# JingyangXiang/LLM-QAT

Hardware: AMD Instinct MI355X
Metric: fake-quant fwd+bwd Gelem/s & achieved HBM GB/s, 4096×11008 bf16 W4A8 (higher is better)
Workload: dtype bf16; 1 GPU; SymQuantizer fwd + STE bwd, W4 on weight-style [4096,11008] + A8 on activation-style [4096,11008], bf16, clip [-2,2] (LLaMA-7B W4-A8 down_proj shapes, configs[1]); parallelism=1gpu

## Files before the change

llm-qat_amd/csrc/fq_dtype_impl.h:

```cpp
#pragma once
#include "../../include/llmqat_fakequant.h"
#include "fq_launch.h"


namespace fq {

#define FQ_LAUNCH(kern, grid, block, st, ...) FQ_LAUNCHK(kern, dim3((unsigned)(grid)), dim3(block), 0, st, __VA_ARGS__)

template <int DT, bool ASYM, bool FAST, bool NTL, int NTS, bool DBG, bool PITCH = false>
static void launch_reg(const RowArgs& a, int64_t nvec, hipStream_t st) {
#define R(TPR, V)                                                                                                   \
    case V:                                                                                                         \
        FQ_LAUNCH((row_reg_kernel<DT, TPR, V, ASYM, FAST, NTL, NTS, DBG, 0, PITCH>), (TPR == 64 ? (a.rows + 3) / 4 : a.rows), \
                  (TPR == 64 ? 256 : TPR), st, a);                                                                  \
        break;
    if (nvec <= 192) {
        switch ((int)((nvec + 63) / 64)) { R(64, 1) R(64, 2) R(64, 3) }
    } else if (nvec <= 384) {
        switch ((int)((nvec + 127) / 128)) { R(128, 2) R(128, 3) }
    } else if (nvec <= 768) {
        switch ((int)((nvec + 255) / 256)) { R(256, 2) R(256, 3) }
    } else if (nvec <= 4096) {
        switch ((int)((nvec + 511) / 512)) { R(512, 2) R(512, 3) R(512, 4) case 5: R(512, 6) case 7: R(512, 8) }
    } else {
        switch ((int)((nvec + 1023) / 1024)) { case 5: R(1024, 6) case 7: R(1024, 8) }
    }
#undef R
}

template <int DT, int AC, bool NTL, bool NTS, bool PITCH = false>
static void launch_reg_ac(const RowArgs& a, int64_t nvec, hipStream_t st) {
#define R(TPR, V)                                                                                                            \
    case V:                                                                                                                  \
        FQ_LAUNCH((row_reg_kernel<DT, TPR, V, false, false, NTL, NTS, false, AC, PITCH>), (TPR == 64 ? (a.rows + 3) / 4 : a.rows),  \
                  (TPR == 64 ? 256 : TPR), st, a);                                                                           \
        break;
    if (nvec <= 192) {
        switch ((int)((nvec + 63) / 64)) { R(64, 1) R(64, 2) R(64, 3) }
    } else if (nvec <= 384) {
        switch ((int)((nvec + 127) / 128)) { R(128, 2) R(128, 3) }
    } else if (nvec <= 768) {
        switch ((int)((nvec + 255) / 256)) { R(256, 2) R(256, 3) }
    } else if (nvec <= 4096) {
        switch ((int)((nvec + 511) / 512)) { R(512, 2) R(512, 3) R(512, 4) case 5: R(512, 6) case 7: R(512, 8) }
    } else {
        switch ((int)((nvec + 1023) / 1024)) { case 5: R(1024, 6) case 7: R(1024, 8) }
    }
#undef R
}

template <int DT, int TPR, bool NTL, bool NTS, bool PITCH = false>
static void launch_wide(const RowArgs& a, int hpt, hipStream_t st) {
    const int64_t grid = TPR == 64 ? (a.rows + 3) / 4 : a.rows;
    constexpr int BLOCK = TPR == 64 ? 256 : TPR;
    const bool mask = any_mask(a) || PITCH;
    switch (hpt) {
#define H(N)                                                                                            \
    case N:                                                                                             \
        if (mask) FQ_LAUNCH((row_reg_wide_kernel<DT, TPR, N, NTL, NTS, true, PITCH>), grid, BLOCK, st, a);     \
        else if constexpr (!PITCH) FQ_LAUNCH((row_reg_wide_kernel<DT, TPR, N, NTL, NTS, false>), grid, BLOCK, st, a);         \
        break;
        H(1) H(2) H(3) H(4) H(5) H(6) case 7: H(8)
#undef H
        default: break;
    }
}

template <int DT, int AC>
static int sym_autocast_t(RowArgs a, void* ws, size_t wsb, hipStream_t st) {
    using T = Ty<DT>;
    begin_launches();
    seal_slots(a);
    if constexpr (T::ESIZE != 2) {
        return fail(FQ_ERR_DTYPE, "autocast arithmetic applies to bf16 / fp16 tensors only");
    } else {
        constexpr int EPV = 8;
        const bool pair = a.n_more > 0;
        const bool vec_ok = aligned16(a.x) && aligned16(a.y) && (a.cols % EPV == 0) && more_aligned(a, 15u, 15u) && pitches_aligned(a, 15, 15);
        const int64_t nvec = a.cols / EPV;
        const int64_t big_rows = largest_rows(a);
        const int64_t bytes = big_rows * a.cols * T::ESIZE;
        if (a.rows > 0x7FFFFFFF) return fail(FQ_ERR_SHAPE, "rows=%lld exceeds the grid limit", (long long)a.rows);
        const bool pitched = any_pitch(a);
        if constexpr (AC == 2) {
            const int64_t nh = a.cols / 4;
            const bool wide_ok = aligned16(a.y) && (reinterpret_cast<uintptr_t>(a.x) & 7u) == 0 && a.cols % 4 == 0 && nh <= 1024 * 8 &&
                                 more_aligned(a, 7u, 15u) && pitches_aligned(a, 7, 15);
            if (wide_ok) {
                const bool ntl = bytes >= NT_LOAD_MIN_BYTES;
#define W(TPR)                                                                                          \
    {                                                                                                   \
        const int hpt = (int)((nh + TPR - 1) / TPR);                                                    \
        if (pitched) launch_wide<DT, TPR, false, true, true>(a, hpt, st);                               \
        else if (ntl) launch_wide<DT, TPR, true, true>(a, hpt, st);                                     \
        else launch_wide<DT, TPR, false, true>(a, hpt, st);                                             \
    }
                if (nh <= 512) W(64) else if (nh <= 2048) W(256) else W(1024)
#undef W
                return launch_result();
            }
            if (pair || a.mask)
                return fail(FQ_ERR_UNSUPPORTED, "fp32-result forward with STE mask / second tensor: rows must be 8-byte aligned, cols %% 4 == 0, cols <= 32768");
            if (a.cols <= GENERIC_MAX_COLS) {
                if (a.cols <= 1024) FQ_LAUNCH((row_generic_kernel<DT, 64, false, AC>), (a.rows + 3) / 4, 256, st, a);
                else FQ_LAUNCH((row_generic_kernel<DT, 256, false, AC>), a.rows, 256, st, a);
                return launch_result();
            }
        } else {
            if (pair && !(vec_ok && nvec <= REG_MAX_VEC))
                return fail(FQ_ERR_UNSUPPORTED, "pair launch: rows must be 16-byte aligned and fit the register kernels");
        }
        if (AC == 1 && vec_ok && nvec <= REG_MAX_VEC) {
            if constexpr (AC == 1) {
                if (pitched) launch_reg_ac<DT, AC, false, true, true>(a, nvec, st);
                else if (bytes >= NT_LOAD_MIN_BYTES) launch_reg_ac<DT, AC, true, true>(a, nvec, st);
                else launch_reg_ac<DT, AC, false, true>(a, nvec, st);
            }
        } else if (a.mask) {
            return fail(FQ_ERR_UNSUPPORTED, "STE-mask forward needs 16-byte aligned rows that fit the register kernels");
        } else if (a.cols <= GENERIC_MAX_COLS) {
            if (a.cols <= 1024) FQ_LAUNCH((row_generic_kernel<DT, 64, false, AC>), (a.rows + 3) / 4, 256, st, a);
            else FQ_LAUNCH((row_generic_kernel<DT, 256, false, AC>), a.rows, 256, st, a);
        } else {
            if (pitched) return fail(FQ_ERR_UNSUPPORTED, "rows that do not follow one another: not served by the two-pass path");
            if (!ws || wsb < (size_t)a.rows * 8)
                return fail(FQ_ERR_WORKSPACE, "two-pass path needs %zu workspace bytes, got %zu", (size_t)a.rows * 8, wsb);
            if (hipMemsetAsync(ws, 0, (size_t)a.rows * 8, st) != hipSuccess) return fail(FQ_ERR_LAUNCH, "hipMemsetAsync failed");
            uint32_t* w = (uint32_t*)ws;
            const bool svec = aligned16(a.x) && a.cols % EPV == 0;
            const int64_t sch = svec ? tp_chunk_elems<DT, true>() : tp_chunk_elems<DT, false>();
            const int64_t schunks = (a.cols + sch - 1) / sch, ach = (int64_t)TP_THREADS * TP_EPT, achunks = (a.cols + ach - 1) / ach;
            if (a.rows * schunks > 0x7FFFFFFF || a.rows * achunks > 0x7FFFFFFF) return fail(FQ_ERR_SHAPE, "rows*chunks exceeds the grid limit");
            if (svec) FQ_LAUNCH((stats_kernel<DT, false, true>), a.rows * schunks, TP_THREADS, st, a, w, schunks);
            else FQ_LAUNCH((stats_kernel<DT, false, false>), a.rows * schunks, TP_THREADS, st, a, w, schunks);
            FQ_LAUNCH((apply_autocast_kernel<DT, AC == 2>), a.rows * achunks, TP_THREADS, st, a, (const uint32_t*)w, achunks);
        }
        return launch_result();
    }
}

template <int DT> int launch_sym_autocast(bool wide, RowArgs a, void* ws, size_t wsb, hipStream_t st) {
    return wide ? sym_autocast_t<DT, 2>(a, ws, wsb, st) : sym_autocast_t<DT, 1>(a, ws, wsb, st);
}

template <int DT, bool ASYM, bool FAST>
static int rowwise_t(RowArgs a, void* ws, size_t wsb, hipStream_t st) {
    using T = Ty<DT>;
    begin_launches();
    seal_slots(a);
    constexpr int EPV = 16 / T::ESIZE;
    const bool pair = a.n_more > 0;
    const bool vec_ok = aligned16(a.x) && aligned16(a.y) && (a.cols % EPV == 0) && more_aligned(a, 15u, 15u) && pitches_aligned(a, 15, 15);
    const int64_t nvec = a.cols / EPV;
    const int64_t big_rows = largest_rows(a);
    const int64_t bytes = big_rows * a.cols * T::ESIZE;
    const bool pitched = any_pitch(a);
    const bool ntl = bytes >= NT_LOAD_MIN_BYTES;
    bool two_pass = false, two_pass_vec = false;
    if (pair && !(vec_ok && nvec <= REG_MAX_VEC)) return fail(FQ_ERR_UNSUPPORTED, "pair launch: rows must be 16-byte aligned and fit the register kernels");
    if (vec_ok && nvec <= REG_MAX_VEC) {
        if (a.rows > 0x7FFFFFFF) return fail(FQ_ERR_SHAPE, "rows=%lld exceeds the grid limit", (long long)a.rows);
        if (a.idx || a.scale) launch_reg<DT, ASYM, FAST, false, false, true>(a, nvec, st);
        else if (pitched) launch_reg<DT, ASYM, FAST, false, true, false, true>(a, nvec, st);
        else if (ntl) launch_reg<DT, ASYM, FAST, true, ASYM ? ST_NT : ST_NT_SC1, false>(a, nvec, st);
        else launch_reg<DT, ASYM, FAST, false, true, false>(a, nvec, st);
    } else if (a.mask) {
        return fail(FQ_ERR_UNSUPPORTED, "STE-mask forward needs 16-byte aligned rows that fit the register kernels");
    } else if (vec_ok && !pitched) {
        two_pass = two_pass_vec = true;
    } else if (a.cols <= GENERIC_MAX_COLS) {
        if (a.rows > 0x7FFFFFFF) return fail(FQ_ERR_SHAPE, "rows=%lld exceeds the grid limit", (long long)a.rows);
        if (a.cols <= 1024) FQ_LAUNCH((row_generic_kernel<DT, 64, ASYM>), (a.rows + 3) / 4, 256, st, a);
        else FQ_LAUNCH((row_generic_kernel<DT, 256, ASYM>), a.rows, 256, st, a);
    } else {
        two_pass = true;
    }
    if (two_pass) {
        if (pitched) return fail(FQ_ERR_UNSUPPORTED, "rows that do not follow one another: not served by the two-pass path");
        if (!ws || wsb < (size_t)a.rows * 8)
// ... 90 lines not shown
    return blk;
}
#define FQ_LAUNCH2(kern, gx_, gy_, block, st, ...) FQ_LAUNCHK(kern, dim3((unsigned)(gx_), (unsigned)(gy_)), dim3(block), 0, st, __VA_ARGS__)

template <int DT> int launch_ste_mask(SteLaunch L, int64_t cols, float lo, float hi, hipStream_t st) {
    using T = Ty<DT>;
    begin_launches();
    constexpr int EPV = 16 / T::ESIZE;
    const int64_t mrw = mask_row_words(cols, T::ESIZE);
    if (!mrw) return fail(FQ_ERR_UNSUPPORTED, "STE-mask backward: shape not served");
    for (int i = 0; i < L.n; ++i)
        if (!(aligned16(L.t[i].g) && aligned16(L.t[i].gx) && (reinterpret_cast<uintptr_t>(L.t[i].mask) & 7u) == 0 && pitch_aligned(L.t[i].gp, 15) &&
              pitch_aligned(L.t[i].op, 15)))
            return fail(FQ_ERR_UNSUPPORTED, "STE-mask backward: alignment not served (g / gx rows 16 bytes, mask 8 bytes)");
    const int64_t nvec_row = cols / EPV;
    const int64_t chunks = (nvec_row + STE_THREADS * 8 - 1) / (STE_THREADS * 8);
    int cv = (int)((nvec_row + chunks - 1) / chunks);
    cv = (cv + 63) / 64 * 64;
    const int vpt = (cv + STE_THREADS - 1) / STE_THREADS;
    const int64_t grid = ste_layout(L, true);
    if (grid > 0x7FFFFFFF) return fail(FQ_ERR_SHAPE, "rows exceed the grid limit");
    int64_t big_rows = 0;
    for (int i = 0; i < L.n; ++i)
        if (!L.t[i].inplace && L.t[i].rows > big_rows) big_rows = L.t[i].rows;
    const int64_t bytes = big_rows * cols * T::ESIZE;
    const bool ntl = bytes >= NT_LOAD_MIN_BYTES;
    bool pitched = false;
    for (int i = 0; i < L.n; ++i) pitched = pitched || L.t[i].gp.on || L.t[i].op.on;
    if (L.n == 1 && !L.t[0].inplace && !pitched) {
        const SteSlot& t0 = L.t[0];
#define S1(V)                                                                                                                                            \
    case V:                                                                                                                                              \
        if (ntl) FQ_LAUNCH2((ste_mask_one_kernel<DT, V, true, true>), grid, chunks, STE_THREADS, st, t0.g, t0.gx, t0.bounds, t0.mask, nvec_row, cv, mrw, lo, hi);   \
        else FQ_LAUNCH2((ste_mask_one_kernel<DT, V, false, true>), grid, chunks, STE_THREADS, st, t0.g, t0.gx, t0.bounds, t0.mask, nvec_row, cv, mrw, lo, hi);      \
        break;
        switch (vpt) { S1(1) S1(2) S1(3) S1(4) S1(5) S1(6) S1(7) S1(8) }
#undef S1
        return launch_result();
    }
    if (L.n <= 2 && !pitched) {
#define S2(V)                                                                                                                  \
    case V:                                                                                                                    \
        if (ntl) FQ_LAUNCH2((ste_mask_kernel<DT, V, true, ST_NT_SC1, false, 2>), grid, chunks, STE_THREADS, st, L, nvec_row, cv, mrw, lo, hi);   \
        else FQ_LAUNCH2((ste_mask_kernel<DT, V, false, true, false, 2>), grid, chunks, STE_THREADS, st, L, nvec_row, cv, mrw, lo, hi);      \
        break;
        switch (vpt) { S2(1) S2(2) S2(3) S2(4) S2(5) S2(6) S2(7) S2(8) }
#undef S2
        return launch_result();
    }
#define S(V)                                                                                                               \
    case V:                                                                                                                \
        if (pitched) FQ_LAUNCH2((ste_mask_kernel<DT, V, false, true, true>), grid, chunks, STE_THREADS, st, L, nvec_row, cv, mrw, lo, hi);   \
        else if (ntl) FQ_LAUNCH2((ste_mask_kernel<DT, V, true, true>), grid, chunks, STE_THREADS, st, L, nvec_row, cv, mrw, lo, hi);        \
        else FQ_LAUNCH2((ste_mask_kernel<DT, V, false, true>), grid, chunks, STE_THREADS, st, L, nvec_row, cv, mrw, lo, hi);           \
        break;
    switch (vpt) { S(1) S(2) S(3) S(4) S(5) S(6) S(7) S(8) }
#undef S
    return launch_result();
}

template <int DT> int launch_ste_mask_wide(SteLaunch L, int64_t cols, float lo, float hi, hipStream_t st) {
    using T = Ty<DT>;
    begin_launches();
    if constexpr (T::ESIZE != 2) {
        return fail(FQ_ERR_DTYPE, "fp32-gradient STE backward applies to bf16 / fp16 inputs only");
    } else {
        const int64_t mrw = mask_row_words(cols, T::ESIZE);
        auto al8 = [](const void* p) { return (reinterpret_cast<uintptr_t>(p) & 7u) == 0; };
        if (!mrw || cols > 32768) return fail(FQ_ERR_UNSUPPORTED, "fp32-gradient STE backward: shape not served");
        for (int i = 0; i < L.n; ++i)
            if (!(aligned16(L.t[i].g) && al8(L.t[i].gx) && al8(L.t[i].mask) && pitch_aligned(L.t[i].gp, 15) && pitch_aligned(L.t[i].op, 7)))
                return fail(FQ_ERR_UNSUPPORTED, "fp32-gradient STE backward: alignment not served");
        const int64_t nh_row = cols / 4;
        const int64_t chunks = (nh_row + STE_THREADS * 8 - 1) / (STE_THREADS * 8);
        int ch = (int)((nh_row + chunks - 1) / chunks);
        ch = (ch + 63) / 64 * 64;
        const int hpt = (ch + STE_THREADS - 1) / STE_THREADS;
        const int64_t grid = ste_layout(L, false);
        if (grid > 0x7FFFFFFF) return fail(FQ_ERR_SHAPE, "rows exceed the grid limit");
        const int64_t bytes = largest_rows(L) * cols * 4;
        const bool ntl = bytes >= NT_LOAD_MIN_BYTES;
        bool pitched = false;
        for (int i = 0; i < L.n; ++i) pitched = pitched || L.t[i].gp.on || L.t[i].op.on;
        if (!ntl && !pitched && L.n <= 2) {
#define SN(V)                                                                                                                                  \
    case V:                                                                                                                                    \
        if (L.n == 1) FQ_LAUNCH2((ste_mask_wide_kernel<DT, V, false, true, false, 1>), grid, chunks, STE_THREADS, st, L, nh_row, ch, mrw, lo, hi);        \
        else FQ_LAUNCH2((ste_mask_wide_kernel<DT, V, false, true, false, 2>), grid, chunks, STE_THREADS, st, L, nh_row, ch, mrw, lo, hi);                 \
        break;
            switch (hpt) { SN(1) SN(2) SN(3) SN(4) SN(5) SN(6) SN(7) SN(8) }
#undef SN
            return launch_result();
        }
#define S(V)                                                                                                                  \
    case V:                                                                                                                   \
        if (pitched) FQ_LAUNCH2((ste_mask_wide_kernel<DT, V, false, true, true>), grid, chunks, STE_THREADS, st, L, nh_row, ch, mrw, lo, hi);   \
        else if (ntl) FQ_LAUNCH2((ste_mask_wide_kernel<DT, V, true, true>), grid, chunks, STE_THREADS, st, L, nh_row, ch, mrw, lo, hi);        \
        else FQ_LAUNCH2((ste_mask_wide_kernel<DT, V, false, true>), grid, chunks, STE_THREADS, st, L, nh_row, ch, mrw, lo, hi);           \
        break;
        switch (hpt) { S(1) S(2) S(3) S(4) S(5) S(6) S(7) S(8) }
#undef S
        return launch_result();
    }
}

template <int DT>
int launch_w12(const void* w, const void* scale, void* out, int64_t rows, int64_t cols, int w_bits, int scale_per_row, float cv,
               hipStream_t st) {
    using T = Ty<DT>;
    begin_launches();
    constexpr int EPV = 16 / T::ESIZE;
    const bool vec = aligned16(w) && aligned16(out) && cols % EPV == 0;
    int64_t grid = vec ? (rows * (cols / EPV) + 255) / 256 : (rows * cols + 255) / 256;
    if (!vec && grid > 16384) grid = 16384;
    if (grid > 0x7FFFFFFF) return fail(FQ_ERR_SHAPE, "tensor too large");
    if (w_bits == 1) {
        if (vec) FQ_LAUNCH((w12_kernel<DT, 1, true>), grid, 256, st, w, scale, out, rows, cols, scale_per_row, cv);
        else FQ_LAUNCH((w12_kernel<DT, 1, false>), grid, 256, st, w, scale, out, rows, cols, scale_per_row, cv);
    } else {
        if (vec) FQ_LAUNCH((w12_kernel<DT, 2, true>), grid, 256, st, w, scale, out, rows, cols, scale_per_row, cv);
        else FQ_LAUNCH((w12_kernel<DT, 2, false>), grid, 256, st, w, scale, out, rows, cols, scale_per_row, cv);
    }
    return launch_result();
}

template <int DT>
int launch_w12_rows(const void* w, void* out, void* scale_out, int64_t rows, int64_t cols, int w_bits, float cv, hipStream_t st) {
    using T = Ty<DT>;
    if (!(aligned16(w) && aligned16(out) && cols % 4 == 0 && cols >= 256 && rows >= 8))
        return fail(FQ_ERR_UNSUPPORTED, "one-launch 1-/2-bit branch: needs rows >= 8, cols >= 256, cols %% 4 == 0 and 16-byte aligned tensors");
    if (rows > 0x7FFFFFFF) return fail(FQ_ERR_SHAPE, "rows=%lld exceeds the grid limit", (long long)rows);
    const int64_t ngroups = cols / 4;
    const bool shared_row = cols >= 8129;
    const int64_t gpt = shared_row ? (ngroups + 511) / 512 : (ngroups + 63) / 64;
    constexpr int MAXG_OWN = DT == F32 ? 16 : 32;
    if (gpt > (shared_row ? 16 : MAXG_OWN) || (shared_row && (cols + 511) / 512 >= 256))
        return fail(FQ_ERR_UNSUPPORTED, "one-launch 1-/2-bit branch: cols=%lld outside the row lengths this kernel holds in registers", (long long)cols);
    begin_launches();
    const float factor = (float)rows / (float)(rows * cols);
    const bool ntl = rows * cols * T::ESIZE >= NT_LOAD_MIN_BYTES;
    const int64_t grid = shared_row ? rows : (rows + 7) / 8;
#define K(SH, G, WB)                                                                                                              \
    {                                                                                                                             \
        if (ntl) FQ_LAUNCH((w12_row_aten_kernel<DT, WB, SH, G, true, true>), grid, 512, st, w, out, scale_out, rows, cols, cv, factor);   \
        else FQ_LAUNCH((w12_row_aten_kernel<DT, WB, SH, G, false, true>), grid, 512, st, w, out, scale_out, rows, cols, cv, factor);      \
    }
#define KW(SH, G)                    \
    {                                \
        if (w_bits == 1) K(SH, G, 1) \
        else K(SH, G, 2)             \
    }
    if (shared_row) {
        if (gpt <= 6) KW(true, 6) else if (gpt <= 8) KW(true, 8) else KW(true, 16)
    } else {
        if (gpt <= 16) KW(false, 16)
        else if constexpr (DT != F32) KW(false, 32)
    }
#undef KW
#undef K
    return launch_result();
}

#define FQ_INSTANTIATE(DT)                                                                                      \
    template int launch_rowwise<DT>(bool, bool, RowArgs, void*, size_t, hipStream_t);                           \
    template int launch_sym_autocast<DT>(bool, RowArgs, void*, size_t, hipStream_t);                                           \
    template int launch_ste<DT>(const void*, const void*, void*, int64_t, float, float, hipStream_t);           \
    template int launch_ste_rows<DT>(const void*, const void*, void*, int64_t, int64_t, float, float, const float*, hipStream_t, const StePitch3&); \
    template int launch_ste_mask<DT>(SteLaunch, int64_t, float, float, hipStream_t);                             \
    template int launch_ste_mask_wide<DT>(SteLaunch, int64_t, float, float, hipStream_t);                        \
    template int launch_w12<DT>(const void*, const void*, void*, int64_t, int64_t, int, int, float, hipStream_t);     \
    template int launch_w12_rows<DT>(const void*, void*, void*, int64_t, int64_t, int, float, hipStream_t);

}
```

llm-qat_amd/csrc/fq_kernels.h:

```cpp
#pragma once
#include "fq_device.h"



namespace fq {

constexpr int MAX_MORE = 3;

struct RowPitch {
    int64_t outer, inner;
    uint32_t n_inner;
    uint32_t on;
};
template <bool PITCH = true> __device__ __forceinline__ int64_t row_byte_off(int64_t row, int64_t row_bytes, const RowPitch& p) {
    if constexpr (!PITCH) {
        return row * row_bytes;
    } else {
        if (!p.on) return row * row_bytes;
        const uint32_t r = (uint32_t)row, q = r / p.n_inner;
        return (int64_t)q * p.outer + (int64_t)(r - q * p.n_inner) * p.inner;
    }
}

struct TensorSlot {
// ... 228 lines not shown
    }

    const bool want_mask = msk && !((ub < a.hi) && (lb > a.lo));
    const bool sym_clip = a.lo == -a.hi;
    const uint32_t clipk = (ub != ub) ? 0u : a.clipk;
    uint8_t* mrow = (uint8_t*)(msk + row * a.mask_row_words);
    int32_t* idxr = (DBG && a.idx) ? a.idx + row * a.cols : nullptr;
#pragma unroll
    for (int i = 0; i < VPT; ++i) {
        const int v = t + i * TPR;
        const uint32_t w[4] = {r[i].x, r[i].y, r[i].z, r[i].w};
        float f[EPV];
#pragma unroll
        for (int d = 0; d < 4; ++d) {
            float fd[T::EPD];
            T::unpack(w[d], fd);
#pragma unroll
            for (int k = 0; k < T::EPD; ++k) f[d * T::EPD + k] = fd[k];
        }
        if (want_mask) ste_mask_record<DT>(mrow, v, v < nvec, r[i], f, a.lo, a.hi, sym_clip, clipk);
        if constexpr (AC != 0) {
#pragma unroll
            for (int e = 0; e < EPV; ++e) f[e] = sym_elem_autocast(f[e], sr);
            uint32_t o[4];
#pragma unroll
            for (int d = 0; d < 4; ++d) {
                float fd[T::EPD];
#pragma unroll
                for (int k = 0; k < T::EPD; ++k) fd[k] = f[d * T::EPD + k];
                o[d] = T::pack(fd);
            }
            if (v < nvec) st16_at<NTS>(yr, v, make_uint4(o[0], o[1], o[2], o[3]));
            continue;
        }
        uint32_t o[4];
        int32_t ib[EPV];
#pragma unroll
        for (int d = 0; d < 4; ++d) {
            float fd[T::EPD];
#pragma unroll
            for (int k = 0; k < T::EPD; ++k) fd[k] = f[d * T::EPD + k];
            int32_t* ip = (DBG && idxr) ? ib + d * T::EPD : nullptr;
            if constexpr (!ASYM) o[d] = sym_chain<DT, FAST>(fd, sr, ip);
            else if constexpr (ALUT) {
                if (use_lut) {
                    const uint16_t* L = lut[TPR == 64 ? (threadIdx.x >> 6) : 0];
                    const uint32_t i0 = as_u(asym_first_half<DT, AFAST>(fd[0], ar, a.asym) + 12582912.0f) & 0xFFu;
                    const uint32_t i1 = as_u(asym_first_half<DT, AFAST>(fd[1], ar, a.asym) + 12582912.0f) & 0xFFu;
                    o[d] = (uint32_t)L[i0] | ((uint32_t)L[i1] << 16);
                } else {
                    o[d] = asym_chain<DT, AFAST>(fd, ar, a.asym, ip);
                }
            } else o[d] = asym_chain<DT, FAST && DT == BF16>(fd, ar, a.asym, ip);
        }
        if (v < nvec) {
            st16_at<NTS>(yr, v, make_uint4(o[0], o[1], o[2], o[3]));
            if constexpr (DBG) {
                if (idxr) {
#pragma unroll
                    for (int e = 0; e < EPV; ++e) idxr[(int64_t)v * EPV + e] = ib[e];
                }
            }
        }
    }
}

typedef uint32_t u32x2_t __attribute__((ext_vector_type(2)));
template <bool NT> __device__ __forceinline__ uint2 ld8(const uint2* p) {
    if constexpr (NT) {
        u32x2_t v = __builtin_nontemporal_load((const u32x2_t*)p);
        return make_uint2(v.x, v.y);
    } else {
        return *p;
    }
}
template <bool NT> __device__ __forceinline__ void st8(uint2* p, uint2 v) {
    if constexpr (NT) {
        u32x2_t w = {v.x, v.y};
        __builtin_nontemporal_store(w, (u32x2_t*)p);
    } else {
        *p = v;
    }
}

template <int DT, int TPR, int HPT, bool NTL, bool NTS, bool MASK, bool PITCH = false>
__global__ __launch_bounds__(TPR == 64 ? 256 : TPR) void row_reg_wide_kernel(RowArgs a) {
    using T = Ty<DT>;
    static_assert(T::ESIZE == 2, "16-bit input, fp32 output");
    constexpr int NW = TPR / 64;
    __shared__ uint32_t red[NW > 1 ? NW : 1];
    int64_t row;
    int t;
    if constexpr (TPR == 64) {
        row = (int64_t)blockIdx.x * 4 + (threadIdx.x >> 6);
        t = threadIdx.x & 63;
        if (row >= a.rows) return;
    } else {
        row = blockIdx.x;
        t = threadIdx.x;
    }
    const void* xb = a.x;
    void* yb = a.y;
    float* bnd = a.bounds;
    uint64_t* msk = a.mask;
    float qmax = a.sym.qmax;
    RowPitch xp = a.xp, yp = a.yp;
    if (row >= a.rows0) {
        int64_t rbase = 0;
#pragma unroll
        for (int i = 0; i < MAX_MORE; ++i) {
            if (i < a.n_more && row >= a.more[i].row_begin) {
                rbase = a.more[i].row_begin;
                xb = a.more[i].x;
                yb = a.more[i].y;
                bnd = a.more[i].bounds;
                msk = a.more[i].mask;
                qmax = a.more[i].qmax;
                if constexpr (PITCH) {
                    xp = a.more[i].xp;
                    yp = a.more[i].yp;
                }
            }
        }
        row -= rbase;
    }
    const int nh = (int)(a.cols / 4);
    const uint2* __restrict__ xr = (const uint2*)((const char*)xb + row_byte_off<PITCH>(row, a.cols * 2, xp));
    uint4* __restrict__ yr = (uint4*)((char*)yb + row_byte_off<PITCH>(row, a.cols * 4, yp));
    uint2 r[HPT];
#pragma unroll
    for (int i = 0; i < HPT; ++i) {
        int h = t + i * TPR;
        h = h < nh ? h : nh - 1;
        r[i] = ld8<NTL>(&xr[h]);
    }
    uint32_t acc = 0;
#pragma unroll
    for (int i = 0; i < HPT; ++i) acc = T::absmax_acc(T::absmax_acc(acc, r[i].x), r[i].y);
    const float m = as_f(block_reduce<OpMaxU, NW>(T::absmax_finish(acc), red));
    const SymRow sr = sym_row_autocast<DT>(m, SymConst{qmax, a.sym.c6});
    if (t == 0 && bnd) {
        bnd[2 * row] = m;
        bnd[2 * row + 1] = -m;
    }
    const bool want_mask = MASK && msk && !((m < a.hi) && (-m > a.lo));
    const bool sym_clip = a.lo == -a.hi;
    const uint32_t clipk = (m != m) ? 0u : a.clipk;
    uint8_t* mrow = (uint8_t*)(msk + row * a.mask_row_words);
#pragma unroll
    for (int i = 0; i < HPT; ++i) {
        const int h = t + i * TPR;
        float f[4];
        {
            float f0[2], f1[2];
            T::unpack(r[i].x, f0);
            T::unpack(r[i].y, f1);
            f[0] = f0[0], f[1] = f0[1], f[2] = f1[0], f[3] = f1[1];
        }
        if (MASK && want_mask) {
            uint32_t nib;
            if (clipk) nib = ste_flags16_pair(r[i].x, r[i].y, clipk);
            else nib = sym_clip ? ste_flags_f<4, true>(f, a.lo, a.hi) : ste_flags_f<4, false>(f, a.lo, a.hi);
            nib = h < nh ? nib : 0u;
            const uint32_t byte = ste_nibble_pair(nib);
            if (h < nh && !(h & 1)) mrow[h >> 1] = (uint8_t)byte;
        }
        const uint4 o = make_uint4(as_u(sym_elem_autocast(f[0], sr)), as_u(sym_elem_autocast(f[1], sr)),
                                   as_u(sym_elem_autocast(f[2], sr)), as_u(sym_elem_autocast(f[3], sr)));
        if (h < nh) st16<NTS>(&yr[h], o);
    }
}

template <int DT, bool FAST> __device__ __forceinline__ float sym_elem(float x, const SymRow& r, int32_t* idx) {
    using T = Ty<DT>;
    float q = __builtin_rintf(T::rb(x * r.s));
    if (idx) *idx = idx_i32(q);
    return FAST ? q * r.rinv : q / r.t2;
}
template <int DT> __device__ __forceinline__ float asym_elem(float x, const AsymRow& r, const AsymConst& k, int32_t* idx) {
    using T = Ty<DT>;
    float n = T::rb(T::rb(x - r.mn) / r.a);
    float q = __builtin_rintf(T::rb(n * k.S));
    if (idx) *idx = idx_i32(q);
    float w = T::rb(k.mul_inv ? q * k.invS : q / k.S);
    return T::rb(w * r.a) + r.mn;
}

template <int DT, int TPR, bool ASYM, int AC = 0>
__global__ __launch_bounds__(TPR == 64 ? 256 : TPR) void row_generic_kernel(RowArgs a) {
    using T = Ty<DT>;
    static_assert(AC == 0 || (!ASYM && T::ESIZE == 2), "autocast arithmetic: Sym on 16-bit tensors");
    constexpr int NW = TPR / 64;
    __shared__ uint32_t red[3][NW > 1 ? NW : 1];
    int64_t row;
    int t;
    if constexpr (TPR == 64) {
        row = (int64_t)blockIdx.x * 4 + (threadIdx.x >> 6);
        t = threadIdx.x & 63;
        if (row >= a.rows) return;
    } else {
        row = blockIdx.x;
        t = threadIdx.x;
    }
    const int64_t base = row * a.cols;
    const int64_t cols = a.cols;
    const int64_t xbase = row_byte_off(row, cols * T::ESIZE, a.xp) / T::ESIZE;
    const int64_t ybase = row_byte_off(row, cols * (AC == 2 ? 4 : T::ESIZE), a.yp) / (AC == 2 ? 4 : T::ESIZE);
    const float first = T::load1(a.x, xbase);
    SymRow sr;
    AsymRow ar;
    if constexpr (!ASYM) {
        uint32_t acc = 0;
        for (int64_t c = t; c < cols; c += TPR) {
            uint32_t b = as_u(T::load1(a.x, xbase + c)) & 0x7FFFFFFFu;
            acc = acc > b ? acc : b;
        }
        const float m = as_f(block_reduce<OpMaxU, NW>(acc, red[0]));
        if constexpr (AC == 0) sr = sym_row<DT>(m, a.sym);
        else sr = sym_row_autocast<DT>(m, a.sym);
        if (t == 0) {
            if (a.scale) a.scale[row] = sr.s;
            if (a.bounds) {
                a.bounds[2 * row] = m;
                a.bounds[2 * row + 1] = -m;
            }
        }
    } else {
        float mx = first, mn = first;
        uint32_t acc = 0;
        for (int64_t c = t; c < cols; c += TPR) {
            float v = T::load1(a.x, xbase + c);
            mx = __builtin_fmaxf(mx, v);
            mn = __builtin_fminf(mn, v);
            uint32_t b = as_u(v) & 0x7FFFFFFFu;
            acc = acc > b ? acc : b;
        }
        const uint32_t nb = block_reduce<OpMaxU, NW>(acc, red[0]);
        mx = as_f(block_reduce<OpMaxF, NW>(as_u(mx), red[1]));
        mn = as_f(block_reduce<OpMinF, NW>(as_u(mn), red[2]));
        if (absbits_is_nan(nb)) mx = mn = as_f(0x7FC00000u);
        ar = asym_row<DT>(mx, mn, a.asym);
        if (t == 0) {
            if (a.scale) {
                a.scale[2 * row] = ar.al;
                a.scale[2 * row + 1] = ar.mn;
            }
            if (a.bounds) {
                a.bounds[2 * row] = mx;
                a.bounds[2 * row + 1] = mn;
            }
        }
    }
// ... 520 lines not shown
                                               int64_t vs, int cv, const float* bounds, float lo, float hi, int t, const RowPitch& gp,
                                               const RowPitch& op) {
    using T = Ty<DT>;
    const uint4* gr = (const uint4*)((const char*)g + row_byte_off<PITCH>(row, nvec_row * 16, gp)) + vs;
    uint4* or_ = (uint4*)((char*)gx + row_byte_off<PITCH>(row, nvec_row * 16, op)) + vs;
    const int64_t rem = nvec_row - vs;
    const int nvec = (int)(rem < cv ? rem : cv);
    uint4 rg[VPT];
#pragma unroll
    for (int i = 0; i < VPT; ++i) {
        int v = t + i * STE_THREADS;
        v = v < nvec ? v : nvec - 1;
        rg[i] = ld16<NTL>(&gr[v]);
    }
    SteMaskHeld<16 / T::ESIZE, VPT> mh;
    mh.load(mrow, vs, mrow_dwords, t);
    bool safe = false;
    if (bounds) {
        const float ub = bounds[2 * row], lb = bounds[2 * row + 1];
        safe = (ub < hi) && (lb > lo);
    }
    if (safe) {
#pragma unroll
        for (int i = 0; i < VPT; ++i) {
            const int v = t + i * STE_THREADS;
            if (v < nvec) st16_at<NTS>(or_, v, rg[i]);
        }
    } else {
        uint32_t mb[VPT];
        mh.bits(t, mb);
#pragma unroll
        for (int i = 0; i < VPT; ++i) {
            const int v = t + i * STE_THREADS;
            const uint4 o = ste_mask_apply<DT>(rg[i], mb[i]);
            if (v < nvec) st16_at<NTS>(or_, v, o);
        }
    }
}

template <int DT, int VPT, bool NTL = true, bool NTS = true>
__global__ __launch_bounds__(STE_THREADS) void ste_mask_one_kernel(const void* g, void* gx, const float* bounds, const uint64_t* mask, int64_t nvec_row, int cv,
                                                                   int64_t mask_row_words, float lo, float hi) {
    const int64_t row = blockIdx.x;
    ste_mask_chunk<DT, VPT, NTL, NTS, false>(g, gx, (const uint8_t*)(mask + row * mask_row_words), (int)mask_row_words * 2, row, nvec_row, (int64_t)blockIdx.y * cv, cv,
                                             bounds, lo, hi, (int)threadIdx.x, RowPitch{}, RowPitch{});
}

template <int DT, int VPT, bool NTL = true, int NTS = ST_NT, bool PITCH = false, int NS = 4>
__global__ __launch_bounds__(STE_THREADS) void ste_mask_kernel(SteLaunch L, int64_t nvec_row, int cv, int64_t mask_row_words, float lo, float hi) {
    __shared__ uint64_t unsafe_rows[STE_THREADS / 64];
    const int t = threadIdx.x;
    const SteSlot sl = ste_pick_slot<PITCH, NS>(L, (int64_t)blockIdx.x);
    const int64_t local = (int64_t)blockIdx.x - sl.blk_begin;
    if (!sl.inplace) {
        ste_mask_chunk<DT, VPT, NTL, NTS, PITCH>(sl.g, sl.gx, (const uint8_t*)(sl.mask + local * mask_row_words), (int)mask_row_words * 2, local, nvec_row,
                                          (int64_t)blockIdx.y * cv, cv, sl.bounds, lo, hi, t, sl.gp, sl.op);
        return;
    }
    if (blockIdx.y) return;
    const int64_t r0 = local * STE_THREADS;
    bool unsafe = false;
    if (r0 + t < sl.rows) {
        const float ub = sl.bounds[2 * (r0 + t)], lb = sl.bounds[2 * (r0 + t) + 1];
        unsafe = !((ub < hi) && (lb > lo));
    }
    const uint64_t bal = __ballot(unsafe);
    if ((t & 63) == 0) unsafe_rows[t >> 6] = bal;
    __syncthreads();
#pragma unroll 1
    for (int w = 0; w < STE_THREADS / 64; ++w) {
        uint64_t bits = unsafe_rows[w];
        while (bits) {
            const int64_t row = r0 + w * 64 + __builtin_ctzll(bits);
            bits &= bits - 1;
            const uint8_t* mrow = (const uint8_t*)(sl.mask + row * mask_row_words);
#pragma unroll 1
            for (int c = 0; c < (int)gridDim.y; ++c)
                ste_mask_chunk<DT, VPT, false, false, PITCH>(sl.g, sl.gx, mrow, (int)mask_row_words * 2, row, nvec_row, (int64_t)c * cv, cv, nullptr, lo, hi, t,
                                                      sl.gp, sl.op);
        }
    }
}

template <int DT, int HPT, bool NTL = true, bool NTS = true, bool PITCH = false, int NS = 4>
__global__ __launch_bounds__(STE_THREADS) void ste_mask_wide_kernel(SteLaunch L, int64_t nh_row, int ch, int64_t mask_row_words, float lo, float hi) {
    using T = Ty<DT>;
    static_assert(T::ESIZE == 2, "fp32 gradient in, 16-bit gradient out");
    typedef short s16x2_t __attribute__((ext_vector_type(2)));
    SteSlot sl;
    if constexpr (NS == 1) sl = L.t[0];
    else sl = ste_pick_slot<PITCH, NS>(L, (int64_t)blockIdx.x);
    const int64_t row = (int64_t)blockIdx.x - sl.blk_begin;
    const int64_t hs = (int64_t)blockIdx.y * ch;
    const uint4* gr = (const uint4*)((const char*)sl.g + row_byte_off<PITCH>(row, nh_row * 16, sl.gp)) + hs;
    uint2* or_ = (uint2*)((char*)sl.gx + row_byte_off<PITCH>(row, nh_row * 8, sl.op)) + hs;
    const int64_t rem = nh_row - hs;
    const int nh = (int)(rem < ch ? rem : ch);
    const int t = threadIdx.x;
    uint4 rg[HPT];
#pragma unroll
    for (int i = 0; i < HPT; ++i) {
        int h = t + i * STE_THREADS;
        h = h < nh ? h : nh - 1;
        rg[i] = ld16<NTL>(&gr[h]);
    }
    SteMaskHeld<4, HPT> mh;
    mh.load((const uint8_t*)(sl.mask + row * mask_row_words), hs, (int)mask_row_words * 2, t);
    const float ub = sl.bounds[2 * row], lb = sl.bounds[2 * row + 1];
    const bool safe = (ub < hi) && (lb > lo);
    uint32_t mb[HPT];
    if (!safe) mh.bits(t, mb);
    else {
#pragma unroll
        for (int i = 0; i < HPT; ++i) mb[i] = 0u;
    }
#pragma unroll
    for (int i = 0; i < HPT; ++i) {
        const int h = t + i * STE_THREADS;
        const float f0[2] = {as_f(rg[i].x), as_f(rg[i].y)}, f1[2] = {as_f(rg[i].z), as_f(rg[i].w)};
        uint32_t w0 = T::pack(f0), w1 = T::pack(f1);
        const uint32_t m2 = mb[i] | (mb[i] << 15);
        w0 &= ~__builtin_bit_cast(uint32_t, __builtin_bit_cast(s16x2_t, m2 << 15) >> (short)15);
        w1 &= ~__builtin_bit_cast(uint32_t, __builtin_bit_cast(s16x2_t, m2 << 13) >> (short)15);
        if (h < nh) st8<NTS>(&or_[h], make_uint2(w0, w1));
    }
}

}
```

Measured before the change: 782.5 Gelem/s.

## Widen fake-quant forward loads and STE backward stores to 16 bytes via lane exchange

Result: no change. 783.5 Gelem/s, median of 6 (+0.1%).

```diff
diff --git a/llm-qat_amd/csrc/fq_dtype_impl.h b/llm-qat_amd/csrc/fq_dtype_impl.h
--- a/llm-qat_amd/csrc/fq_dtype_impl.h
+++ b/llm-qat_amd/csrc/fq_dtype_impl.h
@@ -49,16 +49,42 @@
 #undef R
 }
 
-template <int DT, int TPR, bool NTL, bool NTS, bool PITCH = false>
-static void launch_wide(const RowArgs& a, int hpt, hipStream_t st) {
+#ifndef FQ_WIDE_ST_BIG
+#define FQ_WIDE_ST_BIG ST_NT_SC1
+#endif
+#ifndef FQ_WIDE_ST_SMALL
+#define FQ_WIDE_ST_SMALL ST_NT
+#endif
+
+template <int DT, bool NTL, int NTS, bool PITCH = false>
+static void launch_wide(const RowArgs& a, int64_t nvec, hipStream_t st) {
+    const bool mask = any_mask(a) || PITCH;
+#define R(TPR, V)                                                                                                                          \
+    case V: {                                                                                                                              \
+        const int64_t grid = TPR == 64 ? (a.rows + 3) / 4 : a.rows;                                                                        \
+        if (mask) FQ_LAUNCH((row_reg_wide_kernel<DT, TPR, 2 * V, NTL, NTS, true, PITCH>), grid, (TPR == 64 ? 256 : TPR), st, a);           \
+        else if constexpr (!PITCH) FQ_LAUNCH((row_reg_wide_kernel<DT, TPR, 2 * V, NTL, NTS, false>), grid, (TPR == 64 ? 256 : TPR), st, a); \
+    } break;
+    if (nvec <= 192) {
+        switch ((int)((nvec + 63) / 64)) { R(64, 1) R(64, 2) R(64, 3) }
+    } else if (nvec <= 384) {
+        switch ((int)((nvec + 127) / 128)) { R(128, 2) R(128, 3) }
+    } else if (nvec <= 768) {
+        switch ((int)((nvec + 255) / 256)) { R(256, 2) R(256, 3) }
+    } else {
+        switch ((int)((nvec + 511) / 512)) { R(512, 2) R(512, 3) R(512, 4) case 5: R(512, 6) case 7: R(512, 8) }
+    }
+#undef R
+}
+
+template <int DT, int TPR>
+static void launch_wide_h8(const RowArgs& a, int hpt, hipStream_t st) {
     const int64_t grid = TPR == 64 ? (a.rows + 3) / 4 : a.rows;
     constexpr int BLOCK = TPR == 64 ? 256 : TPR;
-    const bool mask = any_mask(a) || PITCH;
     switch (hpt) {
-#define H(N)                                                                                            \
-    case N:                                                                                             \
-        if (mask) FQ_LAUNCH((row_reg_wide_kernel<DT, TPR, N, NTL, NTS, true, PITCH>), grid, BLOCK, st, a);     \
-        else if constexpr (!PITCH) FQ_LAUNCH((row_reg_wide_kernel<DT, TPR, N, NTL, NTS, false>), grid, BLOCK, st, a);         \
+#define H(N)                                                                                                   \
+    case N:                                                                                                    \
+        FQ_LAUNCH((row_reg_wide_kernel<DT, TPR, N, false, ST_NT, true, true, false>), grid, BLOCK, st, a);     \
         break;
         H(1) H(2) H(3) H(4) H(5) H(6) case 7: H(8)
 #undef H
@@ -88,13 +114,13 @@
                                  more_aligned(a, 7u, 15u) && pitches_aligned(a, 7, 15);
             if (wide_ok) {
                 const bool ntl = bytes >= NT_LOAD_MIN_BYTES;
-#define W(TPR)                                                                                          \
-    {                                                                                                   \
-        const int hpt = (int)((nh + TPR - 1) / TPR);                                                    \
-        if (pitched) launch_wide<DT, TPR, false, true, true>(a, hpt, st);                               \
-        else if (ntl) launch_wide<DT, TPR, true, true>(a, hpt, st);                                     \
-        else launch_wide<DT, TPR, false, true>(a, hpt, st);                                             \
-    }
+                if (a.cols % 8 == 0 && aligned16(a.x) && more_aligned(a, 15u, 15u) && pitches_aligned(a, 15, 15)) {
+                    if (pitched) launch_wide<DT, false, FQ_WIDE_ST_SMALL, true>(a, nvec, st);
+                    else if (ntl) launch_wide<DT, true, FQ_WIDE_ST_BIG>(a, nvec, st);
+                    else launch_wide<DT, false, FQ_WIDE_ST_SMALL>(a, nvec, st);
+                    return launch_result();
+                }
+#define W(TPR) launch_wide_h8<DT, TPR>(a, (int)((nh + TPR - 1) / TPR), st);
                 if (nh <= 512) W(64) else if (nh <= 2048) W(256) else W(1024)
 #undef W
                 return launch_result();
@@ -351,23 +377,35 @@
         const bool ntl = bytes >= NT_LOAD_MIN_BYTES;
         bool pitched = false;
         for (int i = 0; i < L.n; ++i) pitched = pitched || L.t[i].gp.on || L.t[i].op.on;
+        bool x16 = cols % 8 == 0;
+        for (int i = 0; i < L.n; ++i) x16 = x16 && aligned16(L.t[i].gx) && pitch_aligned(L.t[i].op, 15);
+        if (!x16) {
+#define S8(V)                                                                                                                                          \
+    case V:                                                                                                                                            \
+        FQ_LAUNCH2((ste_mask_wide_kernel<DT, V, false, ST_NT, true, 4, false>), grid, chunks, STE_THREADS, st, L, nh_row, ch, mrw, lo, hi);            \
+        break;
+            switch (hpt) { S8(1) S8(2) S8(3) S8(4) S8(5) S8(6) S8(7) S8(8) }
+#undef S8
+            return launch_result();
+        }
+        const int hpt2 = (hpt + 1) / 2 * 2;
         if (!ntl && !pitched && L.n <= 2) {
 #define SN(V)                                                                                                                                  \
     case V:                                                                                                                                    \
-        if (L.n == 1) FQ_LAUNCH2((ste_mask_wide_kernel<DT, V, false, true, false, 1>), grid, chunks, STE_THREADS, st, L, nh_row, ch, mrw, lo, hi);        \
-        else FQ_LAUNCH2((ste_mask_wide_kernel<DT, V, false, true, false, 2>), grid, chunks, STE_THREADS, st, L, nh_row, ch, mrw, lo, hi);                 \
-        break;
-            switch (hpt) { SN(1) SN(2) SN(3) SN(4) SN(5) SN(6) SN(7) SN(8) }
+        if (L.n == 1) FQ_LAUNCH2((ste_mask_wide_kernel<DT, V, false, FQ_WIDE_ST_SMALL, false, 1>), grid, chunks, STE_THREADS, st, L, nh_row, ch, mrw, lo, hi);        \
+        else FQ_LAUNCH2((ste_mask_wide_kernel<DT, V, false, FQ_WIDE_ST_SMALL, false, 2>), grid, chunks, STE_THREADS, st, L, nh_row, ch, mrw, lo, hi);                 \
+        break;
+            switch (hpt2) { SN(2) SN(4) SN(6) SN(8) }
 #undef SN
             return launch_result();
         }
 #define S(V)                                                                                                                  \
     case V:                                                                                                                   \
-        if (pitched) FQ_LAUNCH2((ste_mask_wide_kernel<DT, V, false, true, true>), grid, chunks, STE_THREADS, st, L, nh_row, ch, mrw, lo, hi);   \
-        else if (ntl) FQ_LAUNCH2((ste_mask_wide_kernel<DT, V, true, true>), grid, chunks, STE_THREADS, st, L, nh_row, ch, mrw, lo, hi);        \
-        else FQ_LAUNCH2((ste_mask_wide_kernel<DT, V, false, true>), grid, chunks, STE_THREADS, st, L, nh_row, ch, mrw, lo, hi);           \
-        break;
-        switch (hpt) { S(1) S(2) S(3) S(4) S(5) S(6) S(7) S(8) }
+        if (pitched) FQ_LAUNCH2((ste_mask_wide_kernel<DT, V, false, FQ_WIDE_ST_SMALL, true>), grid, chunks, STE_THREADS, st, L, nh_row, ch, mrw, lo, hi);   \
+        else if (ntl) FQ_LAUNCH2((ste_mask_wide_kernel<DT, V, true, FQ_WIDE_ST_BIG>), grid, chunks, STE_THREADS, st, L, nh_row, ch, mrw, lo, hi);        \
+        else FQ_LAUNCH2((ste_mask_wide_kernel<DT, V, false, FQ_WIDE_ST_SMALL>), grid, chunks, STE_THREADS, st, L, nh_row, ch, mrw, lo, hi);           \
+        break;
+        switch (hpt2) { S(2) S(4) S(6) S(8) }
 #undef S
         return launch_result();
     }
diff --git a/llm-qat_amd/csrc/fq_kernels.h b/llm-qat_amd/csrc/fq_kernels.h
--- a/llm-qat_amd/csrc/fq_kernels.h
+++ b/llm-qat_amd/csrc/fq_kernels.h
@@ -334,11 +334,37 @@
         *p = v;
     }
 }
-
-template <int DT, int TPR, int HPT, bool NTL, bool NTS, bool MASK, bool PITCH = false>
+template <int POL> __device__ __forceinline__ void st8_at(uint2* base , int h, uint2 val) {
+    if constexpr (POL == ST_PLAIN || POL == ST_NT) {
+        st8<POL == ST_NT>(base + h, val);
+    } else {
+        constexpr int AUX = POL == ST_SC1 ? 16 : POL == ST_SC0_SC1 ? 17 : 18;
+        const uint64_t b = (uint64_t)base;
+        const uint64_t bu = (uint64_t)(uint32_t)__builtin_amdgcn_readfirstlane((int)(uint32_t)b) |
+                            ((uint64_t)(uint32_t)__builtin_amdgcn_readfirstlane((int)(uint32_t)(b >> 32)) << 32);
+        const __amdgpu_buffer_rsrc_t rs = __builtin_amdgcn_make_buffer_rsrc((void*)bu, (short)0, 0x7FFFFFFF, 0x00020000);
+        const u32x2_t w = {val.x, val.y};
+        __builtin_amdgcn_raw_buffer_store_b64(w, rs, h * 8, 0, AUX);
+    }
+}
+
+__device__ __forceinline__ void wide_fwd_exchange(const uint4& q, int lane, uint2& h0, uint2& h1) {
+    const bool low = lane < 32, odd = lane & 1;
+    const int near = (lane >> 1) * 4, far = near + 128;
+    const int ab = odd ? far : near, cd = odd ? near : far;
+    const uint32_t A = (uint32_t)__builtin_amdgcn_ds_bpermute(ab, (int)(low ? q.x : q.z));
+    const uint32_t B = (uint32_t)__builtin_amdgcn_ds_bpermute(ab, (int)(low ? q.y : q.w));
+    const uint32_t C = (uint32_t)__builtin_amdgcn_ds_bpermute(cd, (int)(low ? q.z : q.x));
+    const uint32_t D = (uint32_t)__builtin_amdgcn_ds_bpermute(cd, (int)(low ? q.w : q.y));
+    h0 = odd ? make_uint2(C, D) : make_uint2(A, B);
+    h1 = odd ? make_uint2(A, B) : make_uint2(C, D);
+}
+
+template <int DT, int TPR, int HPT, bool NTL, int NTS, bool MASK, bool PITCH = false, bool X16 = true>
 __global__ __launch_bounds__(TPR == 64 ? 256 : TPR) void row_reg_wide_kernel(RowArgs a) {
     using T = Ty<DT>;
     static_assert(T::ESIZE == 2, "16-bit input, fp32 output");
+    static_assert(!X16 || HPT % 2 == 0, "16-byte loads: half-vectors come in pairs");
     constexpr int NW = TPR / 64;
     __shared__ uint32_t red[NW > 1 ? NW : 1];
     int64_t row;
@@ -380,15 +406,38 @@
     const uint2* __restrict__ xr = (const uint2*)((const char*)xb + row_byte_off<PITCH>(row, a.cols * 2, xp));
     uint4* __restrict__ yr = (uint4*)((char*)yb + row_byte_off<PITCH>(row, a.cols * 4, yp));
     uint2 r[HPT];
-#pragma unroll
-    for (int i = 0; i < HPT; ++i) {
-        int h = t + i * TPR;
-        h = h < nh ? h : nh - 1;
-        r[i] = ld8<NTL>(&xr[h]);
-    }
+    int hb[HPT];
     uint32_t acc = 0;
-#pragma unroll
-    for (int i = 0; i < HPT; ++i) acc = T::absmax_acc(T::absmax_acc(acc, r[i].x), r[i].y);
+    if constexpr (X16) {
+        const int nv = nh >> 1, lane = t & 63;
+        uint4 q[HPT / 2];
+#pragma unroll
+        for (int p = 0; p < HPT / 2; ++p) {
+            int v = t + p * TPR;
+            v = v < nv ? v : nv - 1;
+            q[p] = ld16<NTL>((const uint4*)xr + v);
+        }
+#pragma unroll
+        for (int p = 0; p < HPT / 2; ++p) {
+            acc = T::absmax_acc(T::absmax_acc(acc, q[p].x), q[p].y);
+            acc = T::absmax_acc(T::absmax_acc(acc, q[p].z), q[p].w);
+        }
+#pragma unroll
+        for (int p = 0; p < HPT / 2; ++p) {
+            wide_fwd_exchange(q[p], lane, r[2 * p], r[2 * p + 1]);
+            hb[2 * p] = 2 * (p * TPR + (t - lane)) + lane;
+            hb[2 * p + 1] = hb[2 * p] + 64;
+        }
+    } else {
+#pragma unroll
+        for (int i = 0; i < HPT; ++i) {
+            hb[i] = t + i * TPR;
+            const int h = hb[i] < nh ? hb[i] : nh - 1;
+            r[i] = ld8<NTL>(&xr[h]);
+        }
+#pragma unroll
+        for (int i = 0; i < HPT; ++i) acc = T::absmax_acc(T::absmax_acc(acc, r[i].x), r[i].y);
+    }
     const float m = as_f(block_reduce<OpMaxU, NW>(T::absmax_finish(acc), red));
     const SymRow sr = sym_row_autocast<DT>(m, SymConst{qmax, a.sym.c6});
     if (t == 0 && bnd) {
@@ -401,7 +450,7 @@
     uint8_t* mrow = (uint8_t*)(msk + row * a.mask_row_words);
 #pragma unroll
     for (int i = 0; i < HPT; ++i) {
-        const int h = t + i * TPR;
+        const int h = hb[i];
         float f[4];
         {
             float f0[2], f1[2];
@@ -419,7 +468,7 @@
         }
         const uint4 o = make_uint4(as_u(sym_elem_autocast(f[0], sr)), as_u(sym_elem_autocast(f[1], sr)),
                                    as_u(sym_elem_autocast(f[2], sr)), as_u(sym_elem_autocast(f[3], sr)));
-        if (h < nh) st16<NTS>(&yr[h], o);
+        if (h < nh) st16_at<NTS>(yr, h, o);
     }
 }
 
@@ -1106,10 +1155,11 @@
     }
 }
 
-template <int DT, int HPT, bool NTL = true, bool NTS = true, bool PITCH = false, int NS = 4>
+template <int DT, int HPT, bool NTL = true, int NTS = ST_NT, bool PITCH = false, int NS = 4, bool X16 = true>
 __global__ __launch_bounds__(STE_THREADS) void ste_mask_wide_kernel(SteLaunch L, int64_t nh_row, int ch, int64_t mask_row_words, float lo, float hi) {
     using T = Ty<DT>;
     static_assert(T::ESIZE == 2, "fp32 gradient in, 16-bit gradient out");
+    static_assert(!X16 || HPT % 2 == 0, "16-byte stores: slots leave in pairs");
     typedef short s16x2_t __attribute__((ext_vector_type(2)));
     SteSlot sl;
     if constexpr (NS == 1) sl = L.t[0];
@@ -1138,16 +1188,37 @@
 #pragma unroll
         for (int i = 0; i < HPT; ++i) mb[i] = 0u;
     }
+    uint2 w[HPT];
 #pragma unroll
     for (int i = 0; i < HPT; ++i) {
-        const int h = t + i * STE_THREADS;
         const float f0[2] = {as_f(rg[i].x), as_f(rg[i].y)}, f1[2] = {as_f(rg[i].z), as_f(rg[i].w)};
         uint32_t w0 = T::pack(f0), w1 = T::pack(f1);
         const uint32_t m2 = mb[i] | (mb[i] << 15);
         w0 &= ~__builtin_bit_cast(uint32_t, __builtin_bit_cast(s16x2_t, m2 << 15) >> (short)15);
         w1 &= ~__builtin_bit_cast(uint32_t, __builtin_bit_cast(s16x2_t, m2 << 13) >> (short)15);
-        if (h < nh) st8<NTS>(&or_[h], make_uint2(w0, w1));
-    }
-}
-
-}
+        w[i] = make_uint2(w0, w1);
+    }
+    constexpr int NP = X16 ? HPT / 2 : 0;
+    const int lane = t & 63, wbase = t - lane;
+#pragma unroll
+    for (int k = 0; k < NP; ++k) {
+        const bool low = lane < 32, odd = lane & 1;
+        const int s2 = (lane & 31) * 2;
+        const int ab = (low ? s2 : s2 + 1) * 4, cd = (low ? s2 + 1 : s2) * 4;
+        const uint2 a = w[2 * k], b = w[2 * k + 1];
+        const uint32_t A = (uint32_t)__builtin_amdgcn_ds_bpermute(ab, (int)(odd ? b.x : a.x));
+        const uint32_t B = (uint32_t)__builtin_amdgcn_ds_bpermute(ab, (int)(odd ? b.y : a.y));
+        const uint32_t C = (uint32_t)__builtin_amdgcn_ds_bpermute(cd, (int)(odd ? a.x : b.x));
+        const uint32_t D = (uint32_t)__builtin_amdgcn_ds_bpermute(cd, (int)(odd ? a.y : b.y));
+        const uint4 o = low ? make_uint4(A, B, C, D) : make_uint4(C, D, A, B);
+        const int h = wbase + (2 * k + (low ? 0 : 1)) * STE_THREADS + s2;
+        if (h < nh) st16_at<NTS>((uint4*)or_, h >> 1, o);
+    }
+#pragma unroll
+    for (int i = 2 * NP; i < HPT; ++i) {
+        const int h = t + i * STE_THREADS;
+        if (h < nh) st8_at<NTS>(or_, h, w[i]);
+    }
+}
+
+}
```
